# twmitchel/FieldConv

Hardware: AMD Instinct MI355X
Metric: FieldConv fwd+bwd Medges/s (20k verts, k=32, C=48, M=2) (higher is better)
Workload: dtype f32 (complex64 in/out; contractions on f16 MFMA with every operand split into two halves, fp32 accumulate)

## Files before the change

### fieldconv_amd/build.py

```python
import os
import shutil
import subprocess
import sys

PKG = os.path.dirname(os.path.abspath(__file__))
CSRC = os.path.join(PKG, 'csrc')
OUT_DIR = os.path.join(PKG, '_native')
LIB_PATH = os.path.join(OUT_DIR, 'libfieldconv_hip.so')
SOURCES = ['fc_api.hip', 'fc_pack.hip', 'fc_forward.hip', 'fc_forward_split.hip', 'fc_forward_ring.hip', 'fc_backward.hip', 'fc_backward_split.hip', 'fc_generic.hip', 'fc_cgemm.hip', 'fc_wide.hip', 'fc_blocks.hip', 'fc_pointwise.hip', 'fc_pointwise_f64.hip', 'fc_echo.hip', 'fc_trans_field.hip', 'fc_lift_echo_generic.hip', 'fc_head.hip', 'fc_graph.hip', 'fc_precomp.hip', 'fc_optim.hip', 'fc_support.hip', 'fc_loss.hip', 'fc_segment.hip', 'fc_match.hip', 'fc_linear_ce.hip', 'fc_geodesic.hip', 'fc_geodesic_fps.hip', 'fc_logmap.hip', 'fc_mesh_graph.hip', 'fc_transfer.hip', 'fc_norm.hip', 'fc_interp.hip', 'fc_maxpool.hip', 'fc_dropout.hip', 'fc_augment.hip']
HEADERS = ['fc_common.hpp', 'fc_pair.hpp', 'fc_kernels.hpp', 'fc_tile.hpp', 'fc_forward_kernels.hpp', 'fc_forward_ring.hpp', 'fc_backward_kernels.hpp', 'fc_backward_stream.hpp', 'fc_geodesic_relax.hpp', 'fc_segment.hpp', 'fc_select.hpp', 'fc_workspace.hpp', 'fc_philox.hpp', os.path.join('..', '..', 'include', 'fieldconv_hip.h')]
FLAGS = ['-O3', '-std=c++17', '--offload-arch=gfx950', '-fPIC', '-shared', '-fno-slp-vectorize',
         '-fno-gpu-rdc', '-Wno-unused-result']


def _hipcc():
    for cand in (shutil.which('hipcc'), '/opt/rocm/bin/hipcc'):
        if cand and os.path.exists(cand):
            return cand
    raise RuntimeError('hipcc not found: libfieldconv_hip.so cannot be built')


def _source_digest():
    import hashlib
    h = hashlib.sha256()
    for d in [os.path.join(CSRC, s) for s in SOURCES + HEADERS] + [os.path.abspath(__file__)]:
# ... 150 lines not shown
```

### fieldconv_amd/csrc/fc_backward.hip

```cpp
#include <stdio.h>
#include "fc_backward_kernels.hpp"
#include "fc_backward_stream.hpp"

namespace fc {

template <int T>
__global__ __launch_bounds__(kThreads) void fc_backward_filter_kernel(
    const float2* __restrict__ gx_, const float* __restrict__ hdump, float2* __restrict__ ggwp ,
    const BwdArgs a, const int F, const int B) {
    extern __shared__ __attribute__((aligned(16))) char smem[];
    const MmaGeom& mg = a.g;
    const int KD = a.KD, KP = mg.KP, IP = mg.MP, I = a.I;
    float* const slab0 = reinterpret_cast<float*>(smem);
    float* const xtr = slab0 + 2 * a.slab_stride;
    float* const xts = xtr + IP * kXtStride;
    float* const xtd = xts + IP * kXtStride;

    const int tid = threadIdx.x;
    const int lane = tid & 63;
    const int wave = __builtin_amdgcn_readfirstlane(tid >> 6);
    const int f = blockIdx.y;
    const int m = f - B;
    const int fr = lane & 15, fq = lane >> 4;

// ... 490 lines not shown
    }
    const float sc = 1.f / (float)F;
    int r = k / O, o = k - r * O;
    if (pairs == 2) {
        o = k / R;
        r = k - o * R;
    } else if (pairs && k < (R >> 1) * 2 * O) {
        const int pr = k / (2 * O), rem = k - pr * 2 * O;
        r = 2 * pr + (rem & 1);
        o = rem >> 1;
    }
    gw[(((size_t)o * I + i) * R + r) * F + f] = make_float2(s.x * sc, s.y * sc);
}

template <int R, int B>
static int launch_gather(const float2* gy, const float* rec, const fc_csr* g, const float* wpk, char* hrec, const StreamArgs& a,
                         const StreamPlan& p, hipStream_t stream) {
    const size_t lds = (size_t)p.gwpg * kRingChunks * 1024;
    if (p.gwpg == kGatherSmallWaves)
        hipLaunchKernelGGL((fc_backward_gather_kernel<R, B, kGatherSmallWaves, kGatherSmallResidency>), dim3(p.ggrid), dim3(kGatherSmallWaves * kWave),
                           lds, stream, gy, rec, g->rowptr, g->runs, wpk, hrec, a);
    else
        hipLaunchKernelGGL((fc_backward_gather_kernel<R, B, kWaves, kWaves / 4>), dim3(p.ggrid), dim3(kThreads), lds, stream, gy, rec, g->rowptr,
                           g->runs, wpk, hrec, a);
    return hipGetLastError() == hipSuccess ? FC_OK : FC_ERR_LAUNCH;
}

template <int T, int KPT = 0, int IT = 0>
static int launch_stream(const float2* x, const char* hrec, const float* wpk, float2* gwp, float2* gxt, const StreamArgs& a,
                         const StreamPlan& p, hipStream_t stream) {
    auto kern = fc_backward_stream_kernel<T, KPT, IT>;
    static bool lds_ok[kMaxDevices] = {};
    if (!allow_full_lds(reinterpret_cast<const void*>(kern), p.lds, lds_ok)) return FC_ERR_LAUNCH;
    hipLaunchKernelGGL(kern, dim3(p.P, p.FS), dim3(kThreads), p.lds, stream, x, hrec, wpk, gwp, gxt, a);
    return hipGetLastError() == hipSuccess ? FC_OK : FC_ERR_LAUNCH;
}

int backward_stream_impl(const float* x, const float* gy, const float* rec, const fc_csr* g, const float* wpk, float* gx, void* ws,
                         size_t ws_bytes, const fc_dims* d, hipStream_t stream, int stages) {
    const StreamPlan p = plan_stream(d, halves_of(d), true);
    if (!p.ok) return FC_ERR_UNSUPPORTED;
    if (!ws || ws_bytes < p.hrec_bytes + p.gwp_bytes + p.gxt_bytes + p.wst_bytes) return FC_ERR_WORKSPACE;
    StreamArgs a = make_stream_args(d, p);
    char* hrec = static_cast<char*>(ws);
    a.wst = reinterpret_cast<uint32_t*>(hrec + p.hrec_bytes + p.gwp_bytes + p.gxt_bytes);
    float2* gwp = reinterpret_cast<float2*>(hrec + p.hrec_bytes);
    float2* gxt = reinterpret_cast<float2*>(hrec + p.hrec_bytes + p.gwp_bytes);
    const float2* x2 = reinterpret_cast<const float2*>(x);
    int rc = FC_ERR_UNSUPPORTED;
    if (stages & 1) {
        const float2* gy2 = reinterpret_cast<const float2*>(gy);
#define FC_GATHER_CASE(RR, BB) if (d->R == RR && d->B == BB) rc = launch_gather<RR, BB>(gy2, rec, g, wpk, hrec, a, p, stream);
        FC_GATHER_CASE(2, 1) FC_GATHER_CASE(4, 1) FC_GATHER_CASE(6, 1) FC_GATHER_CASE(8, 1)
        FC_GATHER_CASE(2, 2) FC_GATHER_CASE(4, 2) FC_GATHER_CASE(6, 2) FC_GATHER_CASE(8, 2)
        FC_GATHER_CASE(2, 3) FC_GATHER_CASE(4, 3) FC_GATHER_CASE(6, 3) FC_GATHER_CASE(8, 3)
#undef FC_GATHER_CASE
        if (rc != FC_OK) return rc;
    }
    if (!(stages & 2)) return FC_OK;
    if (p.T == 6 && p.KPS == 288 && d->I == 48) rc = launch_stream<6, 288, 48>(x2, hrec, wpk, gwp, gxt, a, p, stream);
    else if (p.T == 6 && p.KPS == 192 && d->I == 64) rc = launch_stream<6, 192, 64>(x2, hrec, wpk, gwp, gxt, a, p, stream);
    else if (p.T <= 2) rc = launch_stream<2>(x2, hrec, wpk, gwp, gxt, a, p, stream);
    else if (p.T <= 4) rc = launch_stream<4>(x2, hrec, wpk, gwp, gxt, a, p, stream);
    else rc = launch_stream<6>(x2, hrec, wpk, gwp, gxt, a, p, stream);
    if (rc != FC_OK || (stages & 4)) return rc;
    const size_t count = (size_t)d->N * d->I;
    const dim3 grid((unsigned)((count + 255) / 256));
    float2* gx2 = reinterpret_cast<float2*>(gx);
    if (d->B == 1) hipLaunchKernelGGL(fc_backward_gx_kernel<1>, grid, dim3(256), 0, stream, x2, gxt, gx2, count, p.KS);
    else if (d->B == 2) hipLaunchKernelGGL(fc_backward_gx_kernel<2>, grid, dim3(256), 0, stream, x2, gxt, gx2, count, p.KS);
    else hipLaunchKernelGGL(fc_backward_gx_kernel<3>, grid, dim3(256), 0, stream, x2, gxt, gx2, count, p.KS);
    return hipGetLastError() == hipSuccess ? FC_OK : FC_ERR_LAUNCH;
}

bool backward_streams(const fc_dims* d, bool factored) { return plan_stream(d, halves_of(d), factored).ok; }

bool backward_fits(const fc_dims* d) { return plan_backward(d, halves_of(d)).ok_factored; }

size_t backward_workspace_bytes(const fc_dims* d) {
    const BwdPlan p = plan_backward(d, halves_of(d));
    const size_t pair = p.hdump_bytes + p.gwp_bytes + p.gxp_bytes + 256;
    const StreamPlan sp = plan_stream(d, halves_of(d), true);
    const size_t stream = sp.ok ? sp.hrec_bytes + sp.gwp_bytes + sp.gxt_bytes + sp.wst_bytes + 256 : 0;
    return pair > stream ? pair : stream;
}

template <int T>
static int launch_backward_filter(const float2* x, const float* hdump, float2* gwp, const BwdArgs& a, const BwdPlan& p,
                                  const fc_dims* d, hipStream_t stream) {
    static const bool half2 = !(dev_env("FC_FILTER2") && atoi(dev_env("FC_FILTER2")) == 0);
    static bool ok_half2[kMaxDevices] = {}, ok_half[kMaxDevices] = {}, ok_f32[kMaxDevices] = {};
    if (p.fhalf && half2) {
        const size_t lds2 = (size_t)(2 * kTile * filter_image_stride(p.KP) + 2 * 6 * p.IP * kXbStride + 8) * sizeof(_Float16) + 16;
        static bool ok_half2h[kMaxDevices] = {};
        if (a.dump_halves) {
            if (!allow_full_lds(reinterpret_cast<const void*>(fc_backward_filter_half2_kernel<T, true>), lds2, ok_half2h)) return FC_ERR_LAUNCH;
            hipLaunchKernelGGL((fc_backward_filter_half2_kernel<T, true>), dim3(p.P, p.F), dim3(kThreads), lds2, stream, x, hdump, gwp, a, p.F,
                               d->B, d->R * d->O);
// ... 28 lines not shown
        const int per_col = kWaves / p.g.NMT, row_tiles = p.KP / 16;
        need = (row_tiles + per_col - 1) / per_col;
    }
    if (need <= 2) return launch_backward_filter<2>(x2, hdump, gwp, a, p, d, stream);
    if (need <= 4) return launch_backward_filter<4>(x2, hdump, gwp, a, p, d, stream);
    if (need <= 6) return launch_backward_filter<6>(x2, hdump, gwp, a, p, d, stream);
    if (need <= kMaxGwTiles) return launch_backward_filter<kMaxGwTiles>(x2, hdump, gwp, a, p, d, stream);
    return FC_ERR_UNSUPPORTED;
}

void describe_backward(const fc_dims* d, int records, char* buf, size_t n) {
    {
        const StreamPlan sp = plan_stream(d, halves_of(d), records != 0);
        if (sp.ok) {
            snprintf(buf, n, "fc_backward_gather_kernel<records,split-f16> tiles=%d (%d workgroups of %d wavefronts, %d per SIMD); fc_backward_stream_kernel (H once for gxt and gW: %d gxt + %d gW "
                     "wavefronts, W_f in registers, records by LDS-DMA) grid=%dx%d; fc_backward_gx_kernel; module parameters: "
                     "fc_backward_finish_params (sum of the partials + parameter chain) in one launch; explicit filter: fc_backward_finish; cus=%d",
                     sp.ntiles, sp.ggrid, sp.gwpg, sp.gwaves, sp.G, sp.NW, sp.P, sp.FS, num_cus());
            return;
        }
    }
    const BwdPlan p = plan_backward(d, halves_of(d));
    const char* mode = halves_of(d) == 2 ? "split-f16" : halves_of(d) == 1 ? "f16" : "f32";
    static const bool staged = [] { const char* e = dev_env("FC_FILTER2"); return e && atoi(e) == 0; }();
    static const bool split_finish = [] { const char* e = dev_env("FC_SPLIT_FINISH"); return e && atoi(e) != 0; }();
    const int gx_parts = (1 << p.parts_log2) * (p.gsplit ? 2 : 1);
    char fin[320];
    if (split_finish)
        snprintf(fin, sizeof(fin), "%sfc_backward_finish + fc_filter_param_grads (two launches: the split-finish development switch)",
                 gx_parts > 1 ? "fc_sum_parts_kernel (the partial gx arrays), " : "");
    else
// ... 72 lines not shown
```

### fieldconv_amd/csrc/fc_backward_stream.hpp

```cpp
#pragma once
#include <stdlib.h>
#include "fc_backward_kernels.hpp"

namespace fc {

constexpr int kStreamUnits = 4;
constexpr int kStreamPartStride = 2 * kTile + 4;

struct StreamPlan {
    bool ok;
    int F, KP, IP, NMT, KST, KSI, NU, G, NW, T, ntiles, P, nslots;
    int KS;
    int FS, KPS;
    int NG;
    int gwpg, gwaves;
    int ggrid;
    int img_bytes;
    int rec_bytes;
    size_t lds;
    size_t hrec_bytes, gwp_bytes, gxt_bytes, wst_bytes;
    int nt_dump;
};

struct StreamArgs {
    int N, I, O, R, F, B;
    int KP, IP, NMT, KST, KSI, G, NW, ntiles, P, nslots;
    int KS;
    int img_bytes, rec_bytes;
    int wKI, wKP;
    int nt_dump;
    uint32_t* wst;
    unsigned long long* stamps;
    unsigned long long* meter;
    int dbg;
};

constexpr int kGatherSmallWaves = 4;
constexpr int kGatherSmallResidency = 5;
inline void plan_gather(const fc_dims* d, StreamPlan& p);

inline StreamPlan plan_stream(const fc_dims* d, int halves, bool factored) {
    StreamPlan p = {};
    p.ok = false;
    static const bool off = [] { const char* e = dev_env("FC_BWD_STREAM"); return e && atoi(e) == 0; }();
    if (off || !factored || halves != 2 || d->N <= 0) return p;
    const int R = d->R, O = d->O, I = d->I;
// ... 27 lines not shown
    const int cus = num_cus();
    if (4 * p.ntiles < 3 * cus) return p;
    p.P = cus / p.FS;
    if (p.P < 1) p.P = 1;
    p.img_bytes = kTile * p.KSI * 2;
    p.rec_bytes = round_up(p.img_bytes + 2 * kTile * 4, 1024);
    if (I & 1) return p;
    p.lds = (size_t)2 * p.rec_bytes + (size_t)2 * 4 * p.IP * kXbStride * 2 + (size_t)3 * kTile * I * 8 + 4 * 64 * 4 + 2 * 8 * 64 * 4 +
            2 * 64 * 4 + (size_t)2 * p.nslots * kTile * kStreamPartStride * 4;
    if (kTile * I * 8 > kWaves * 1024 - 1024) return p;
    if ((size_t)d->N * I * 8 >= ((size_t)1 << 32)) return p;
    if (p.lds > kMaxLds) return p;
    p.hrec_bytes = (size_t)p.ntiles * p.FS * p.rec_bytes + 1024;
    p.gwp_bytes = (size_t)p.P * p.F * p.KP * p.IP * sizeof(float2);
    p.gxt_bytes = (size_t)p.FS * d->N * I * sizeof(float2);
    p.wst_bytes = (size_t)p.FS * p.G * 4 * kStreamUnits * kWave * 16;
    p.nt_dump = p.hrec_bytes > ((size_t)192 << 20) ? 1 : 0;
    plan_gather(d, p);
    p.ok = true;
    return p;
}

inline StreamArgs make_stream_args(const fc_dims* d, const StreamPlan& p) {
    StreamArgs a;
    a.N = d->N; a.I = d->I; a.O = d->O; a.R = d->R; a.F = p.FS; a.B = d->B; a.KS = p.KS;
    a.KP = p.KPS; a.IP = p.IP; a.NMT = p.NMT; a.KST = p.KST; a.KSI = p.KSI; a.G = p.G; a.NW = p.NW; a.ntiles = p.ntiles; a.P = p.P;
    a.nslots = p.nslots;
    a.img_bytes = p.img_bytes; a.rec_bytes = p.rec_bytes;
    const MmaGeom gw = make_mma_geom(d->I, d->R, d->O, 2);
    a.wKI = gw.KI; a.wKP = gw.KP;
    a.nt_dump = p.nt_dump;
    a.wst = nullptr;
    static const int dbg = [] { const char* e = dev_env("FC_DEBUG_BWD"); return e ? atoi(e) : 0; }();
    a.dbg = dbg;
    static const bool stamp_me = [] { const char* e = dev_env("FC_STAMP_KERNEL"); return e && e[0] == 's'; }();
    a.stamps = stamp_me ? debug_stamp_buffer() : nullptr;
    static const bool meter_me = [] { const char* e = dev_env("FC_STAMP_KERNEL"); return e && e[0] == 'w'; }();
    a.meter = meter_me && debug_stamp_buffer() ? debug_stamp_buffer() + kMeterGather : nullptr;
    return a;
}

typedef uint32_t u32x3 __attribute__((ext_vector_type(3)));

template <int R, bool NT>
__device__ __forceinline__ void store_plane_row(uint32_t* dst, const uint32_t (&w)[R / 2]) {
    if constexpr (R == 2) {
        if (NT) __builtin_nontemporal_store(w[0], dst); else *dst = w[0];
// ... 3 lines not shown
        if (NT) __builtin_nontemporal_store(v, reinterpret_cast<u2*>(dst)); else *reinterpret_cast<u2*>(dst) = v;
    } else if constexpr (R == 6) {
        typedef u32x3 __attribute__((aligned(4))) u3;
        const u32x3 v = {w[0], w[1], w[2]};
        if (NT) __builtin_nontemporal_store(v, reinterpret_cast<u3*>(dst)); else *reinterpret_cast<u3*>(dst) = v;
    } else {
        typedef u32x4 __attribute__((aligned(4))) u4;
        const u32x4 v = {w[0], w[1], w[2], w[3]};
        if (NT) __builtin_nontemporal_store(v, reinterpret_cast<u4*>(dst)); else *reinterpret_cast<u4*>(dst) = v;
    }
}

template <int R, int B, int WPG, int MINW>
__global__ __launch_bounds__(WPG * kWave, MINW) void fc_backward_gather_kernel(
    const float2* __restrict__ ggy, const float* __restrict__ gsten, const int32_t* __restrict__ growptr,
    const int32_t* __restrict__ gruns, const float* __restrict__ gwpk, char* __restrict__ hrec, const StreamArgs a) {
    constexpr int F = 2 * B + 1;
    static_assert(F * R <= 64 && (R & 1) == 0, "at most two walks per vertex, an even ring count");
    constexpr int NG = (F * R + 31) / 32;
    constexpr int FG = (F + NG - 1) / NG;
    constexpr int RECF = factored_record_floats(B);
    constexpr int LOG_CR = factored_log_chunk_records(B);
    constexpr int CR = 1 << LOG_CR;
    constexpr int NR = kRingChunks;
    extern __shared__ __attribute__((aligned(16))) char smem[];
    const int tid = threadIdx.x;
    const int lane = tid & 63;
    const int wave = __builtin_amdgcn_readfirstlane(tid >> 6);
    float* const ring = reinterpret_cast<float*>(smem) + wave * NR * 256;
    const int O = a.O;
    const int ol = lane < O ? lane : 0;

    auto dma_chunk = [&](const int first, const int ch) {
        uint32_t lane_off = lane;
        asm volatile("" : "+v"(lane_off));
        const char* src = reinterpret_cast<const char*>(gsten + ((size_t)first + ((size_t)ch << LOG_CR)) * RECF) + lane_off * 16u;
        __builtin_amdgcn_global_load_lds((gptr_t)src, (lptr_t)(ring + (ch & (NR - 1)) * 256), 16, 0, 0);
    };
    auto slot_range = [&](const int item, int& b, int& e, int (&run)[R]) {
        b = 0;
        e = 0;
#pragma unroll
        for (int q = 0; q < R; ++q) run[q] = 0;
// ... 160 lines not shown
                        float* tail = reinterpret_cast<float*>(recf + half_off + (uint32_t)a.img_bytes);
                        tail[row] = scale;
                        tail[kTile + row] = inv_scale;
                    }
                }
            };
            if (a.nt_dump && !(kDevSwitches && (a.dbg & 32))) rows(std::true_type{}); else rows(std::false_type{});
        });
        beg = nbeg;
        end = nend;
#pragma unroll
        for (int q = 0; q < R; ++q) ro[q] = nro[q];
    }

    meter.close();

    {
        const int total = a.F * a.G * kStreamUnits * 4 * kWave;
        const int NU = a.NMT * a.KST;
        const size_t plane_sz = (size_t)a.IP * a.wKP;
        const uint16_t* const img0 = reinterpret_cast<const uint16_t*>(gwpk + a.IP);
        for (int e = (blockIdx.x * WPG + wave) * kWave + lane; e < total; e += gridDim.x * (WPG * kWave)) {
            const int ln = e & 63, pl = (e >> 6) & 3, ui = (e >> 8) % kStreamUnits, fg = e / (kStreamUnits * 4 * kWave);
            const int g_ = fg % a.G, sl = fg / a.G;
            const int f_ = sl / a.KS, k0 = (sl - f_ * a.KS) * a.KP;
            const int fr_ = ln & 15, fq_ = ln >> 4;
            const int u = min(g_ * kStreamUnits + ui, NU - 1);
            const int mt = u / a.KST, kb = u - mt * a.KST;
            const int row = (mt * 16 + fr_) * 32;
            const uint16_t* const img = img0 + ((size_t)f_ * 4 + pl) * plane_sz;
            int o = (k0 + kb * 32 + 8 * fq_) / R, r = k0 + kb * 32 + 8 * fq_ - o * R;
            uint32_t v[4];
#pragma unroll
            for (int jj = 0; jj < 4; ++jj) {
                uint32_t pr[2];
#pragma unroll
                for (int e2 = 0; e2 < 2; ++e2) {
                    const int kk = r * a.wKI + o;
                    pr[e2] = img[(size_t)(kk >> 5) * a.IP * 32 + row + (kk & 31)];
                    if (++r == R) { r = 0; ++o; }
                }
                v[jj] = pr[0] | (pr[1] << 16);
            }
            *reinterpret_cast<u32x4*>(a.wst + (size_t)e * 4) = u32x4{v[0], v[1], v[2], v[3]};
        }
    }
}

template <int R, int B>
inline bool gather_fits_small() {
    static const bool fits = [] {
        hipFuncAttributes at;
        const void* fn = reinterpret_cast<const void*>(fc_backward_gather_kernel<R, B, kGatherSmallWaves, kGatherSmallResidency>);
        if (hipFuncGetAttributes(&at, fn) != hipSuccess) {
            (void)hipGetLastError();
            return false;
        }
        return at.localSizeBytes == 0 && at.numRegs <= (512 / kGatherSmallResidency) / 8 * 8;
    }();
    return fits;
}
// ... 197 lines not shown
        stamp(10);
        asm volatile("s_waitcnt vmcnt(0) lgkmcnt(0)" ::: "memory");
        stamp(0);
        __builtin_amdgcn_s_barrier();
        stamp(2);
        requests(k + 1, k + 3, a.G);
        stamp(4);
        stamp(1);
    };

    if (is_gxt) {
        const int u0 = wave * kStreamUnits;
        const int NU = a.NMT * a.KST;
        u32x4 wrh[kStreamUnits], wrl[kStreamUnits], wih[kStreamUnits], wil[kStreamUnits];
        {
            const u32x4* const ws = reinterpret_cast<const u32x4*>(a.wst) + (size_t)(f * a.G + wave) * (kStreamUnits * 4 * kWave) + lane;
#pragma unroll
            for (int ui = 0; ui < kStreamUnits; ++ui) {
                wrh[ui] = ws[(ui * 4 + 0) * kWave];
                wrl[ui] = ws[(ui * 4 + 1) * kWave];
                wih[ui] = ws[(ui * 4 + 2) * kWave];
                wil[ui] = ws[(ui * 4 + 3) * kWave];
            }
        }
        first_requests();
#pragma unroll
        for (int ui = 0; ui < kStreamUnits; ++ui) asm volatile("" : "+v"(wrh[ui]), "+v"(wrl[ui]), "+v"(wih[ui]), "+v"(wil[ui]));
        const int hbase = fr * KSI + 8 * fq;
        for (int k = 0; k < nrec; ++k) {
            head(k);
            if (k > 0) reduce_gxt(k - 1);
            const lds_f16* const img = (const lds_f16*)(smem + (k & 1) * a.rec_bytes) + hbase;
            if (!(kDevSwitches && (a.dbg & 2))) {
                float* const pp = part0 + (k & 1) * part_floats + (4 * fq) * kStreamPartStride + 2 * fr;
                const float isv = tail0[(k & 3) * 64 + kTile + fr];
                f32x4 are = {0.f, 0.f, 0.f, 0.f}, aim = are, arn = are;
                int mt_prev = u0 / a.KST;
// ... 152 lines not shown
```

### fieldconv_amd/csrc/fc_kernels.hpp

```cpp
#pragma once
#include <hip/hip_runtime.h>
#include "../../include/fieldconv_hip.h"

#define FC_FOR_EACH_SHAPE(X) \
    X(2, 1) X(3, 1) X(4, 1) X(5, 1) X(6, 1) X(7, 1) X(8, 1) \
    X(2, 2) X(3, 2) X(4, 2) X(5, 2) X(6, 2) X(7, 2) X(8, 2) \
    X(2, 3) X(3, 3) X(4, 3) X(5, 3) X(6, 3) X(7, 3) X(8, 3)

namespace fc {

constexpr size_t kMaxLds = 160 * 1024;
constexpr int kDefaultCUs = 256;
constexpr int kMaxDevices = 16;
inline int num_cus() {
    static int cached[kMaxDevices] = {};
    int dev = 0;
    if (hipGetDevice(&dev) != hipSuccess || dev < 0) return kDefaultCUs;
    if (dev < kMaxDevices && cached[dev] > 0) return cached[dev];
    int n = 0;
    if (hipDeviceGetAttribute(&n, hipDeviceAttributeMultiprocessorCount, dev) != hipSuccess || n <= 0) n = kDefaultCUs;
    if (dev < kMaxDevices) cached[dev] = n;
    return n;
}
constexpr int kMaxChannels = 64;

int forward_impl(const float* x, const float* sten, const fc_csr* g, const float* wpk, float* y,
                 const fc_dims* d, int kind, void* ws, size_t ws_bytes, const fc_epilogue* epi, hipStream_t stream);
size_t forward_workspace_bytes(const fc_dims* d, int kind);
size_t backward_workspace_bytes(const fc_dims* d);
int backward_data_impl(const float* x, const float* gy, const float* sten, const fc_csr* g, const float* wpk, float* gx,
                       void* ws, size_t ws_bytes, const fc_dims* d, bool factored, hipStream_t stream, bool defer_gx_sum = false);
int backward_filter_impl(const float* x, void* ws, size_t ws_bytes, const fc_dims* d, hipStream_t stream, bool factored = false);
bool backward_streams(const fc_dims* d, bool factored);
int backward_stream_impl(const float* x, const float* gy, const float* rec, const fc_csr* g, const float* wpk, float* gx, void* ws,
                         size_t ws_bytes, const fc_dims* d, hipStream_t stream, int stages);
int backward_finish_impl(float* gw_eff, void* ws, size_t ws_bytes, const fc_dims* d, hipStream_t stream, bool factored = false);
int pack_filter_impl(const float* w_eff, float* wpk_fwd, float* wpk_bwd, const fc_dims* d, int records, hipStream_t stream);
int pack_filter_params_impl(const float* zonal, const float* sph, const float* phase, int ftype, float* wpk_fwd,
                            float* wpk_bwd, const fc_dims* d, int records, hipStream_t stream);
int pack_filter_params_pair_impl(const fc_filter_params& f0, float* fwd0, float* bwd0, const fc_dims* d0, const fc_filter_params& f1,
                                 float* fwd1, float* bwd1, const fc_dims* d1, int records, hipStream_t stream);
size_t packed_filter_floats_fwd(const fc_dims* d, int records);
size_t packed_filter_floats_bwd(const fc_dims* d, int records);

bool ring_enabled(const fc_dims* d);
bool forward_ring_fits(const fc_dims* d);
size_t packed_ring_image_floats(int M, int F, int channels, int R, int halves);
int forward_ring_impl(const float* x, const float* rec, const fc_csr* g, const float* wpk, float* y, const fc_dims* d, int kind,
// ... 49 lines not shown
```

### fieldconv_amd/csrc/fc_pack.hip

```cpp
#include <stdlib.h>
#include "fc_common.hpp"
#include "fc_kernels.hpp"
#include "fc_tile.hpp"
#include "fc_forward_ring.hpp"

namespace fc {

__device__ __forceinline__ float2 filter_entry(const float* __restrict__ zonal, const float* __restrict__ sph,
                                               const float* __restrict__ phase, int ftype, int B, int R, int I, int o, int i,
                                               int r, int f) {
    const size_t oir = ((size_t)o * I + i) * R + r;
    if (ftype == 2) {
        if (f == B) return make_float2(zonal[oir * 2], zonal[oir * 2 + 1]);
        const int b = f < B ? f : f - 1;
        const float* p = sph + (oir * (2 * B) + b) * 2;
        return make_float2(p[0], p[1]);
    }
    const int q = f >= B ? f - B : B - f;
    const float z = zonal[oir];
    float2 sp = make_float2(0.f, 0.f);
    if (B > 0) sp = *reinterpret_cast<const float2*>(sph + (oir * B + (q > 0 ? q - 1 : 0)) * 2);
    float ph = 0.f;
    if (ftype == 1) ph = phase[((size_t)o * I + i) * (B + 1) + q];
    float2 c = q == 0 ? make_float2(z, 0.f) : make_float2(sp.x, f > B ? sp.y : -sp.y);
    if (ftype == 1) {
        float s, co;
        sincosf(ph, &s, &co);
        c = cmul(c, make_float2(co, s));
    }
    return c;
}

struct PackArgs {
    int O, I, R, F, B, ftype;
    MmaGeom gf, gb;
    unsigned blocks_f;
    int ring_f;
    int o0, i0, Ifull;
};

constexpr int kPackThreads = 256;

template <bool FROM_PARAMS, bool WITH_PHASE>
__device__ __forceinline__ float2 packed_value(const float2* __restrict__ w, const float* __restrict__ zonal,
                                               const float* __restrict__ sph, const float* __restrict__ phase,
                                               const PackArgs& a, bool is_bwd, int m, int k, int slab) {
    const int KI = is_bwd ? a.gb.KI : a.gf.KI;
    const bool ring = !is_bwd && a.ring_f;
    const int kk = k / KI, c = k - kk * KI;
    const int r = ring ? slab : kk, f = ring ? kk : slab;
    if (f >= a.F) return make_float2(0.f, 0.f);
    const int o = is_bwd ? c : m, i = is_bwd ? m : c;
    if (o >= a.O || i >= a.I || r >= a.R) return make_float2(0.f, 0.f);
    const float2 v = FROM_PARAMS ? filter_entry(zonal, sph, phase, (!WITH_PHASE && a.ftype == 1) ? 0 : a.ftype, a.B, a.R, a.Ifull, a.o0 + o,
                                                a.i0 + i, r, f)
                                 : w[(((size_t)(a.o0 + o) * a.Ifull + a.i0 + i) * a.R + r) * a.F + f];
// ... 46 lines not shown
    const unsigned blk = is_bwd ? block - a.blocks_f : block;
    const MmaGeom& g = is_bwd ? a.gb : a.gf;
    float* const img = is_bwd ? bwd : fwd;
    if (!g.split) {
        const size_t j = (size_t)blk * kPackThreads + threadIdx.x;
        if (j >= (size_t)a.F * 2 * g.MP * g.KP) return;
        const int k = j % g.KP;
        const int m = (j / g.KP) % g.MP;
        const int pl = (j / ((size_t)g.KP * g.MP)) % 2;
        const int f = j / ((size_t)g.KP * g.MP * 2);
        const float2 v = packed_value<FROM_PARAMS, true>(w, zonal, sph, phase, a, is_bwd, m, k, f);
        img[j] = pl == 0 ? v.x : v.y;
        return;
    }
    __shared__ float red[kPackThreads / kWave];
    const int nslab = (!is_bwd && a.ring_f) ? a.R : a.F;
    const int m = blk / nslab, f = blk - m * nslab;
    float mx = row_max2<FROM_PARAMS>(w, zonal, sph, a, is_bwd, m);
#pragma unroll
    for (int d = 32; d >= 1; d >>= 1) mx = fmaxf(mx, __shfl_xor(mx, d, 64));
    if ((threadIdx.x & 63) == 0) red[threadIdx.x >> 6] = mx;
    __syncthreads();
    mx = sqrtf(fmaxf(fmaxf(red[0], red[1]), fmaxf(red[2], red[3]))) * 1.0000002f;
    float scale, inv;
    split_scale(mx, scale, inv);
    if (threadIdx.x == 0 && f == 0) img[m] = inv;
    _Float16* const planes = reinterpret_cast<_Float16*>(img + g.MP);
    const size_t plane = (size_t)g.MP * g.KP;
    for (int k = threadIdx.x; k < g.KP; k += kPackThreads) {
        const float2 v = packed_value<FROM_PARAMS, true>(w, zonal, sph, phase, a, is_bwd, m, k, f);
        _Float16 rh, rl, ih, il;
        split_halves(v.x * scale, rh, rl);
        split_halves(v.y * scale, ih, il);
        _Float16* p = planes + (size_t)f * 2 * g.split * plane + ((size_t)(k >> 5) * g.MP + m) * 32 + (k & 31);
        if (g.split == 2) {
            p[0] = rh;
            p[plane] = rl;
            p[2 * plane] = ih;
            p[3 * plane] = il;
        } else {
            p[0] = rh;
            p[plane] = ih;
        }
    }
}

template <bool FROM_PARAMS>
__global__ __launch_bounds__(kPackThreads) void fc_pack_filter_kernel(const float2* __restrict__ w, const float* __restrict__ zonal,
                                                                      const float* __restrict__ sph,
                                                                      const float* __restrict__ phase, float* __restrict__ fwd,
                                                                      float* __restrict__ bwd, const PackArgs a) {
    pack_filter_body<FROM_PARAMS>(w, zonal, sph, phase, fwd, bwd, a, blockIdx.x);
}

struct PackPtrs { const float* zonal; const float* sph; const float* phase; float* fwd; float* bwd; };
__global__ __launch_bounds__(kPackThreads) void fc_pack_filter_pair_kernel(const PackPtrs p0, const PackArgs a0, const PackPtrs p1,
                                                                           const PackArgs a1, const unsigned split) {
    if (blockIdx.x < split) pack_filter_body<true>(nullptr, p0.zonal, p0.sph, p0.phase, p0.fwd, p0.bwd, a0, blockIdx.x);
    else pack_filter_body<true>(nullptr, p1.zonal, p1.sph, p1.phase, p1.fwd, p1.bwd, a1, blockIdx.x - split);
// ... 8 lines not shown
size_t packed_filter_floats_fwd(const fc_dims* d, int records) {
    if (ring_forward_image(d, records)) return packed_ring_image_floats(d->O, 2 * d->B + 1, d->I, d->R, halves_of(d));
    return packed_image_floats(d->O, d->R, d->I, 2 * d->B + 1, halves_of(d));
}
size_t packed_filter_floats_bwd(const fc_dims* d, int records) {
    (void)records;
    return packed_image_floats(d->I, d->R, d->O, 2 * d->B + 1, halves_of(d));
}

static unsigned pack_args(PackArgs& a, int ftype, bool want_fwd, bool want_bwd, const fc_dims* d, int records, int o0, int i0, int Ifull) {
    a.O = d->O; a.I = d->I; a.R = d->R; a.B = d->B; a.F = 2 * d->B + 1; a.ftype = ftype;
    a.o0 = o0; a.i0 = i0; a.Ifull = Ifull > 0 ? Ifull : d->I;
    a.ring_f = ring_forward_image(d, records & 1) ? 1 : 0;
    a.gf = a.ring_f ? ring_geom(d->O, a.F, d->I, halves_of(d)) : make_mma_geom(d->O, d->R, d->I, halves_of(d));
    a.gb = make_mma_geom(d->I, d->R, d->O, halves_of(d));
    a.blocks_f = want_fwd ? pack_blocks(a.gf, a.ring_f ? a.R : a.F) : 0u;
    const unsigned blocks_b = pack_blocks(a.gb, a.F);
    return a.blocks_f + (want_bwd ? blocks_b : 0u);
}

int pack_filter_params_pair_impl(const fc_filter_params& f0, float* fwd0, float* bwd0, const fc_dims* d0, const fc_filter_params& f1,
                                 float* fwd1, float* bwd1, const fc_dims* d1, int records, hipStream_t stream) {
    PackArgs a0, a1;
    const unsigned n0 = pack_args(a0, f0.ftype, fwd0 != nullptr, bwd0 != nullptr, d0, records, 0, 0, 0);
    const unsigned n1 = pack_args(a1, f1.ftype, fwd1 != nullptr, bwd1 != nullptr, d1, records, 0, 0, 0);
    if (n0 == 0 || n1 == 0) return FC_ERR_BAD_ARGUMENT;
    const PackPtrs p0{f0.zonal, f0.spherical, f0.phase, fwd0, bwd0}, p1{f1.zonal, f1.spherical, f1.phase, fwd1, bwd1};
    hipLaunchKernelGGL(fc_pack_filter_pair_kernel, dim3(n0 + n1), dim3(kPackThreads), 0, stream, p0, a0, p1, a1, n0);
    return hipGetLastError() == hipSuccess ? FC_OK : FC_ERR_LAUNCH;
}
// ... 247 lines not shown
```

### fieldconv_amd/functional.py

```python
import ctypes
import os

import torch

from . import _lib
from ._launch import NO_GUARD as _NO_GUARD, _dp, _p, _po, by_value as _by_value, carve as _carve, on as _on, scratch as _scratch, stream as _stream
from ._lib import FcCsr, FcDims, FcEpilogue, FcFilterParams, check


class KernelTimer:

    def __init__(self):
        self.enabled = False
        self.stride = 1
        self.events = {}
        self.count = {}
        self.pool = []

    def reset(self, pairs=0):
        self.events = {}
        self.count = {}
        self.pool = [(torch.cuda.Event(enable_timing=True), torch.cuda.Event(enable_timing=True)) for _ in range(pairs)]

    def elapsed_ms(self):
# ... 94 lines not shown
@_lib.keep_mode
class _FieldConvFn(torch.autograd.Function):

    @staticmethod
    def forward(ctx, x, w_eff, graph):
        lib = _lib.load()
        x = _by_value(x)
        w_eff = _by_value(w_eff)
        O, I, R, F = w_eff.shape
        B = (F - 1) // 2
        plan = _conv_plan(lib, graph, I, O, B)
        with _on(x.device):
            st = _stream()

            def pack(pl, wpk_f, wpk_b):
                check(lib.fc_pack_filter(_p(w_eff), _p(wpk_f), _po(wpk_b), pl.dref, pl.records, st), 'fc_pack_filter')
            y, wpk_b = _run_forward(lib, x, graph, plan, O, st, pack)
        ctx.save_for_backward(x, wpk_b)
        ctx.graph = graph
        ctx.wshape = (O, I, R, F)
        return y

    @staticmethod
    def backward(ctx, gy):
        lib = _lib.load()
        x, wpk_b = ctx.saved_tensors
        O, I, R, F = ctx.wshape
        plan = _conv_plan(lib, ctx.graph, I, O, (F - 1) // 2)
        gy = _by_value(gy)
        with _on(x.device):
            gx, gw, _ = _launch_backward(lib, x, gy, ctx.graph, wpk_b, plan, ctx.wshape, _stream())
# ... 95 lines not shown
            kind, recs, _ = _records(graph)
            check(lib.fc_forward_params(_p(x), _p(recs), plan.cref_t, kind, ctypes.byref(_filter_params(params)), _p(wpk_f), _p(wpk_b), _p(y),
                                        _po(ws), plan.ws_fwd, plan.dref, plan.records, epi, st), 'fc_forward_params')
            return (y if bias is None else (y, act)), wpk_b
        pack(plan, wpk_f, wpk_b)
        if between is not None:
            between()
        return _launch_forward(lib, x, graph, wpk_f, plan, O, st, addend=addend, bias=bias), wpk_b
    y = torch.empty((nt, O), dtype=torch.complex64, device=dev)
    act = torch.empty_like(y) if bias is not None else None
    if len(ranges) == 1 and between is not None:
        between()
    for row0, nrows in ranges:
        sub = _row_plan(lib, graph, plan, row0, nrows)
        wpk_f = torch.empty(sub.n_fwd, dtype=torch.float32, device=dev)
        pack(sub, wpk_f, wpk_b if row0 == 0 else None)
        _launch_forward(lib, x, graph, wpk_f, sub, O, st, addend=addend, bias=bias, out=(y, act), row0=row0)
        if row0 == 0 and len(ranges) == 2:
            between()
    return (y if bias is None else (y, act)), wpk_b


def _param_grads(params):
    zonal, spherical, phase, ftype = params
    return torch.empty_like(zonal), torch.empty_like(spherical), (torch.empty_like(phase) if ftype == 1 else None)


def _launch_backward(lib, x, gy, graph, wpk_b, plan, wshape, st, params=None, bias_sum=None):
    O, I, R, F = wshape
    gx = torch.empty_like(x)
    want_gw = params is None or KEEP_GW_EFF or _split_finish()
# ... 31 lines not shown
    if graph.on_gx is not None:
        graph.on_gx(gx)
    with _timed('fc_backward_filter'):
        check(lib.fc_backward_filter(_p(x), wsp, nbytes, plan.dref, plan.records, st), 'fc_backward_filter')
    if fp is not None:
        check(lib.fc_backward_finish_params(gwp, wsp, nbytes, plan.dref, plan.records, ctypes.byref(fp), st), 'fc_backward_finish_params')
    else:
        check(lib.fc_backward_finish(_p(gw), wsp, nbytes, plan.dref, plan.records, st), 'fc_backward_finish')
    return gx, gw, pgrads


def _param_packer(lib, params, st):
    zonal, spherical, phase, ftype = params

    def pack(pl, wpk_f, wpk_b):
        check(lib.fc_pack_filter_params(_p(zonal), _p(spherical), _p(phase), ftype, _p(wpk_f), _po(wpk_b), pl.dref, pl.records, st),
              'fc_pack_filter_params')
    return pack


@_lib.keep_mode
class _FieldConvParamFn(torch.autograd.Function):

    @staticmethod
    def forward(ctx, x, zonal, spherical, phase, ftype, B, graph):
        lib = _lib.load()
        x = _by_value(x)
        zonal, spherical, phase = _by_value(zonal), _by_value(spherical, 8), _by_value(phase)
        O, I, R = zonal.shape[0], zonal.shape[1], zonal.shape[2]
        F = 2 * B + 1
        plan = _conv_plan(lib, graph, I, O, B)
# ... 695 lines not shown
```

Baseline: 1824.

## Write backward filter fragments in MMA order during packing, drop gather-kernel reshuffle

The filter-packing kernel now stages the backward split-f16 planes in LDS and writes them directly in the per-lane fragment order that the backward stream kernel loads into registers. The gather kernel no longer carries a tail loop that rebuilt this fragment table from the packed image on every backward pass. The stream kernel reads the fragments straight from the packed filter buffer. This removes scattered 16-bit reads and an extra workspace write from backward, in exchange for LDS staging and an extra pack call for the backward filter when rows are split.

```diff
diff --git a/fieldconv_amd/build.py b/fieldconv_amd/build.py
--- a/fieldconv_amd/build.py
+++ b/fieldconv_amd/build.py
@@ -8,7 +8,7 @@
 OUT_DIR = os.path.join(PKG, '_native')
 LIB_PATH = os.path.join(OUT_DIR, 'libfieldconv_hip.so')
 SOURCES = ['fc_api.hip', 'fc_pack.hip', 'fc_forward.hip', 'fc_forward_split.hip', 'fc_forward_ring.hip', 'fc_backward.hip', 'fc_backward_split.hip', 'fc_generic.hip', 'fc_cgemm.hip', 'fc_wide.hip', 'fc_blocks.hip', 'fc_pointwise.hip', 'fc_pointwise_f64.hip', 'fc_echo.hip', 'fc_trans_field.hip', 'fc_lift_echo_generic.hip', 'fc_head.hip', 'fc_graph.hip', 'fc_precomp.hip', 'fc_optim.hip', 'fc_support.hip', 'fc_loss.hip', 'fc_segment.hip', 'fc_match.hip', 'fc_linear_ce.hip', 'fc_geodesic.hip', 'fc_geodesic_fps.hip', 'fc_logmap.hip', 'fc_mesh_graph.hip', 'fc_transfer.hip', 'fc_norm.hip', 'fc_interp.hip', 'fc_maxpool.hip', 'fc_dropout.hip', 'fc_augment.hip']
-HEADERS = ['fc_common.hpp', 'fc_pair.hpp', 'fc_kernels.hpp', 'fc_tile.hpp', 'fc_forward_kernels.hpp', 'fc_forward_ring.hpp', 'fc_backward_kernels.hpp', 'fc_backward_stream.hpp', 'fc_geodesic_relax.hpp', 'fc_segment.hpp', 'fc_select.hpp', 'fc_workspace.hpp', 'fc_philox.hpp', os.path.join('..', '..', 'include', 'fieldconv_hip.h')]
+HEADERS = ['fc_common.hpp', 'fc_pair.hpp', 'fc_kernels.hpp', 'fc_tile.hpp', 'fc_forward_kernels.hpp', 'fc_forward_ring.hpp', 'fc_backward_kernels.hpp', 'fc_backward_stream.hpp', 'fc_stream_frag.hpp', 'fc_geodesic_relax.hpp', 'fc_segment.hpp', 'fc_select.hpp', 'fc_workspace.hpp', 'fc_philox.hpp', os.path.join('..', '..', 'include', 'fieldconv_hip.h')]
 FLAGS = ['-O3', '-std=c++17', '--offload-arch=gfx950', '-fPIC', '-shared', '-fno-slp-vectorize',
          '-fno-gpu-rdc', '-Wno-unused-result']
 
diff --git a/fieldconv_amd/csrc/fc_backward.hip b/fieldconv_amd/csrc/fc_backward.hip
--- a/fieldconv_amd/csrc/fc_backward.hip
+++ b/fieldconv_amd/csrc/fc_backward.hip
@@ -528,15 +528,15 @@
 }
 
 template <int R, int B>
-static int launch_gather(const float2* gy, const float* rec, const fc_csr* g, const float* wpk, char* hrec, const StreamArgs& a,
+static int launch_gather(const float2* gy, const float* rec, const fc_csr* g, char* hrec, const StreamArgs& a,
                          const StreamPlan& p, hipStream_t stream) {
     const size_t lds = (size_t)p.gwpg * kRingChunks * 1024;
     if (p.gwpg == kGatherSmallWaves)
         hipLaunchKernelGGL((fc_backward_gather_kernel<R, B, kGatherSmallWaves, kGatherSmallResidency>), dim3(p.ggrid), dim3(kGatherSmallWaves * kWave),
-                           lds, stream, gy, rec, g->rowptr, g->runs, wpk, hrec, a);
+                           lds, stream, gy, rec, g->rowptr, g->runs, hrec, a);
     else
         hipLaunchKernelGGL((fc_backward_gather_kernel<R, B, kWaves, kWaves / 4>), dim3(p.ggrid), dim3(kThreads), lds, stream, gy, rec, g->rowptr,
-                           g->runs, wpk, hrec, a);
+                           g->runs, hrec, a);
     return hipGetLastError() == hipSuccess ? FC_OK : FC_ERR_LAUNCH;
 }
 
@@ -554,17 +554,17 @@
                          size_t ws_bytes, const fc_dims* d, hipStream_t stream, int stages) {
     const StreamPlan p = plan_stream(d, halves_of(d), true);
     if (!p.ok) return FC_ERR_UNSUPPORTED;
-    if (!ws || ws_bytes < p.hrec_bytes + p.gwp_bytes + p.gxt_bytes + p.wst_bytes) return FC_ERR_WORKSPACE;
+    if (!ws || ws_bytes < p.hrec_bytes + p.gwp_bytes + p.gxt_bytes + p.spare_bytes) return FC_ERR_WORKSPACE;
     StreamArgs a = make_stream_args(d, p);
     char* hrec = static_cast<char*>(ws);
-    a.wst = reinterpret_cast<uint32_t*>(hrec + p.hrec_bytes + p.gwp_bytes + p.gxt_bytes);
+    a.wst = reinterpret_cast<const uint32_t*>(wpk + stream_frag_offset_floats(d));
     float2* gwp = reinterpret_cast<float2*>(hrec + p.hrec_bytes);
     float2* gxt = reinterpret_cast<float2*>(hrec + p.hrec_bytes + p.gwp_bytes);
     const float2* x2 = reinterpret_cast<const float2*>(x);
     int rc = FC_ERR_UNSUPPORTED;
     if (stages & 1) {
         const float2* gy2 = reinterpret_cast<const float2*>(gy);
-#define FC_GATHER_CASE(RR, BB) if (d->R == RR && d->B == BB) rc = launch_gather<RR, BB>(gy2, rec, g, wpk, hrec, a, p, stream);
+#define FC_GATHER_CASE(RR, BB) if (d->R == RR && d->B == BB) rc = launch_gather<RR, BB>(gy2, rec, g, hrec, a, p, stream);
         FC_GATHER_CASE(2, 1) FC_GATHER_CASE(4, 1) FC_GATHER_CASE(6, 1) FC_GATHER_CASE(8, 1)
         FC_GATHER_CASE(2, 2) FC_GATHER_CASE(4, 2) FC_GATHER_CASE(6, 2) FC_GATHER_CASE(8, 2)
         FC_GATHER_CASE(2, 3) FC_GATHER_CASE(4, 3) FC_GATHER_CASE(6, 3) FC_GATHER_CASE(8, 3)
@@ -589,13 +589,19 @@
 
 bool backward_streams(const fc_dims* d, bool factored) { return plan_stream(d, halves_of(d), factored).ok; }
 
+bool backward_stream_frag(const fc_dims* d, bool factored, StreamFrag* frag) {
+    const StreamPlan p = plan_stream(d, halves_of(d), factored);
+    if (p.ok && frag) *frag = p.frag;
+    return p.ok;
+}
+
 bool backward_fits(const fc_dims* d) { return plan_backward(d, halves_of(d)).ok_factored; }
 
 size_t backward_workspace_bytes(const fc_dims* d) {
     const BwdPlan p = plan_backward(d, halves_of(d));
     const size_t pair = p.hdump_bytes + p.gwp_bytes + p.gxp_bytes + 256;
     const StreamPlan sp = plan_stream(d, halves_of(d), true);
-    const size_t stream = sp.ok ? sp.hrec_bytes + sp.gwp_bytes + sp.gxt_bytes + sp.wst_bytes + 256 : 0;
+    const size_t stream = sp.ok ? sp.hrec_bytes + sp.gwp_bytes + sp.gxt_bytes + sp.spare_bytes + 256 : 0;
     return pair > stream ? pair : stream;
 }
 
@@ -654,7 +660,7 @@
         const StreamPlan sp = plan_stream(d, halves_of(d), records != 0);
         if (sp.ok) {
             snprintf(buf, n, "fc_backward_gather_kernel<records,split-f16> tiles=%d (%d workgroups of %d wavefronts, %d per SIMD); fc_backward_stream_kernel (H once for gxt and gW: %d gxt + %d gW "
-                     "wavefronts, W_f in registers, records by LDS-DMA) grid=%dx%d; fc_backward_gx_kernel; module parameters: "
+                     "wavefronts, W_f in registers from the fragment-order filter the packing launch wrote, records by LDS-DMA) grid=%dx%d; fc_backward_gx_kernel; module parameters: "
                      "fc_backward_finish_params (sum of the partials + parameter chain) in one launch; explicit filter: fc_backward_finish; cus=%d",
                      sp.ntiles, sp.ggrid, sp.gwpg, sp.gwaves, sp.G, sp.NW, sp.P, sp.FS, num_cus());
             return;
diff --git a/fieldconv_amd/csrc/fc_backward_stream.hpp b/fieldconv_amd/csrc/fc_backward_stream.hpp
--- a/fieldconv_amd/csrc/fc_backward_stream.hpp
+++ b/fieldconv_amd/csrc/fc_backward_stream.hpp
@@ -1,10 +1,10 @@
 #pragma once
 #include <stdlib.h>
 #include "fc_backward_kernels.hpp"
+#include "fc_stream_frag.hpp"
 
 namespace fc {
 
-constexpr int kStreamUnits = 4;
 constexpr int kStreamPartStride = 2 * kTile + 4;
 
 struct StreamPlan {
@@ -18,7 +18,9 @@
     int img_bytes;
     int rec_bytes;
     size_t lds;
-    size_t hrec_bytes, gwp_bytes, gxt_bytes, wst_bytes;
+    size_t hrec_bytes, gwp_bytes, gxt_bytes;
+    StreamFrag frag;
+    size_t spare_bytes;
     int nt_dump;
 };
 
@@ -29,7 +31,8 @@
     int img_bytes, rec_bytes;
     int wKI, wKP;
     int nt_dump;
-    uint32_t* wst;
+    const uint32_t* wst;
+    StreamFrag frag;
     unsigned long long* stamps;
     unsigned long long* meter;
     int dbg;
@@ -87,7 +90,8 @@
     p.hrec_bytes = (size_t)p.ntiles * p.FS * p.rec_bytes + 1024;
     p.gwp_bytes = (size_t)p.P * p.F * p.KP * p.IP * sizeof(float2);
     p.gxt_bytes = (size_t)p.FS * d->N * I * sizeof(float2);
-    p.wst_bytes = (size_t)p.FS * p.G * 4 * kStreamUnits * kWave * 16;
+    p.frag = StreamFrag{R, p.FS, p.KS, p.KPS, p.KST, p.NU};
+    p.spare_bytes = (size_t)p.FS * p.G * 4 * kStreamUnits * kWave * 16;
     p.nt_dump = p.hrec_bytes > ((size_t)192 << 20) ? 1 : 0;
     plan_gather(d, p);
     p.ok = true;
@@ -104,6 +108,7 @@
     a.wKI = gw.KI; a.wKP = gw.KP;
     a.nt_dump = p.nt_dump;
     a.wst = nullptr;
+    a.frag = p.frag;
     static const int dbg = [] { const char* e = dev_env("FC_DEBUG_BWD"); return e ? atoi(e) : 0; }();
     a.dbg = dbg;
     static const bool stamp_me = [] { const char* e = dev_env("FC_STAMP_KERNEL"); return e && e[0] == 's'; }();
@@ -137,7 +142,7 @@
 template <int R, int B, int WPG, int MINW>
 __global__ __launch_bounds__(WPG * kWave, MINW) void fc_backward_gather_kernel(
     const float2* __restrict__ ggy, const float* __restrict__ gsten, const int32_t* __restrict__ growptr,
-    const int32_t* __restrict__ gruns, const float* __restrict__ gwpk, char* __restrict__ hrec, const StreamArgs a) {
+    const int32_t* __restrict__ gruns, char* __restrict__ hrec, const StreamArgs a) {
     constexpr int F = 2 * B + 1;
     static_assert(F * R <= 64 && (R & 1) == 0, "at most two walks per vertex, an even ring count");
     constexpr int NG = (F * R + 31) / 32;
@@ -147,9 +152,8 @@
     constexpr int CR = 1 << LOG_CR;
     constexpr int NR = kRingChunks;
     extern __shared__ __attribute__((aligned(16))) char smem[];
-    const int tid = threadIdx.x;
-    const int lane = tid & 63;
-    const int wave = __builtin_amdgcn_readfirstlane(tid >> 6);
+    const int lane = threadIdx.x & 63;
+    const int wave = __builtin_amdgcn_readfirstlane(threadIdx.x >> 6);
     float* const ring = reinterpret_cast<float*>(smem) + wave * NR * 256;
     const int O = a.O;
     const int ol = lane < O ? lane : 0;
@@ -340,37 +344,6 @@
     }
 
     meter.close();
-
-    {
-        const int total = a.F * a.G * kStreamUnits * 4 * kWave;
-        const int NU = a.NMT * a.KST;
-        const size_t plane_sz = (size_t)a.IP * a.wKP;
-        const uint16_t* const img0 = reinterpret_cast<const uint16_t*>(gwpk + a.IP);
-        for (int e = (blockIdx.x * WPG + wave) * kWave + lane; e < total; e += gridDim.x * (WPG * kWave)) {
-            const int ln = e & 63, pl = (e >> 6) & 3, ui = (e >> 8) % kStreamUnits, fg = e / (kStreamUnits * 4 * kWave);
-            const int g_ = fg % a.G, sl = fg / a.G;
-            const int f_ = sl / a.KS, k0 = (sl - f_ * a.KS) * a.KP;
-            const int fr_ = ln & 15, fq_ = ln >> 4;
-            const int u = min(g_ * kStreamUnits + ui, NU - 1);
-            const int mt = u / a.KST, kb = u - mt * a.KST;
-            const int row = (mt * 16 + fr_) * 32;
-            const uint16_t* const img = img0 + ((size_t)f_ * 4 + pl) * plane_sz;
-            int o = (k0 + kb * 32 + 8 * fq_) / R, r = k0 + kb * 32 + 8 * fq_ - o * R;
-            uint32_t v[4];
-#pragma unroll
-            for (int jj = 0; jj < 4; ++jj) {
-                uint32_t pr[2];
-#pragma unroll
-                for (int e2 = 0; e2 < 2; ++e2) {
-                    const int kk = r * a.wKI + o;
-                    pr[e2] = img[(size_t)(kk >> 5) * a.IP * 32 + row + (kk & 31)];
-                    if (++r == R) { r = 0; ++o; }
-                }
-                v[jj] = pr[0] | (pr[1] << 16);
-            }
-            *reinterpret_cast<u32x4*>(a.wst + (size_t)e * 4) = u32x4{v[0], v[1], v[2], v[3]};
-        }
-    }
 }
 
 template <int R, int B>
@@ -598,13 +571,14 @@
         const int NU = a.NMT * a.KST;
         u32x4 wrh[kStreamUnits], wrl[kStreamUnits], wih[kStreamUnits], wil[kStreamUnits];
         {
-            const u32x4* const ws = reinterpret_cast<const u32x4*>(a.wst) + (size_t)(f * a.G + wave) * (kStreamUnits * 4 * kWave) + lane;
+            const u32x4* const ws = reinterpret_cast<const u32x4*>(a.wst) + stream_frag_entry(a.frag, f, 0, 0, lane);
 #pragma unroll
             for (int ui = 0; ui < kStreamUnits; ++ui) {
-                wrh[ui] = ws[(ui * 4 + 0) * kWave];
-                wrl[ui] = ws[(ui * 4 + 1) * kWave];
-                wih[ui] = ws[(ui * 4 + 2) * kWave];
-                wil[ui] = ws[(ui * 4 + 3) * kWave];
+                const u32x4* const wu = ws + stream_frag_step(stream_frag_slot_unit(a.frag, wave, ui), 0);
+                wrh[ui] = wu[stream_frag_step(0, 0)];
+                wrl[ui] = wu[stream_frag_step(0, 1)];
+                wih[ui] = wu[stream_frag_step(0, 2)];
+                wil[ui] = wu[stream_frag_step(0, 3)];
             }
         }
         first_requests();
diff --git a/fieldconv_amd/csrc/fc_kernels.hpp b/fieldconv_amd/csrc/fc_kernels.hpp
--- a/fieldconv_amd/csrc/fc_kernels.hpp
+++ b/fieldconv_amd/csrc/fc_kernels.hpp
@@ -32,6 +32,8 @@
                        void* ws, size_t ws_bytes, const fc_dims* d, bool factored, hipStream_t stream, bool defer_gx_sum = false);
 int backward_filter_impl(const float* x, void* ws, size_t ws_bytes, const fc_dims* d, hipStream_t stream, bool factored = false);
 bool backward_streams(const fc_dims* d, bool factored);
+struct StreamFrag;
+bool backward_stream_frag(const fc_dims* d, bool factored, StreamFrag* frag);
 int backward_stream_impl(const float* x, const float* gy, const float* rec, const fc_csr* g, const float* wpk, float* gx, void* ws,
                          size_t ws_bytes, const fc_dims* d, hipStream_t stream, int stages);
 int backward_finish_impl(float* gw_eff, void* ws, size_t ws_bytes, const fc_dims* d, hipStream_t stream, bool factored = false);
diff --git a/fieldconv_amd/csrc/fc_pack.hip b/fieldconv_amd/csrc/fc_pack.hip
--- a/fieldconv_amd/csrc/fc_pack.hip
+++ b/fieldconv_amd/csrc/fc_pack.hip
@@ -3,6 +3,7 @@
 #include "fc_kernels.hpp"
 #include "fc_tile.hpp"
 #include "fc_forward_ring.hpp"
+#include "fc_stream_frag.hpp"
 
 namespace fc {
 
@@ -36,10 +37,14 @@
     MmaGeom gf, gb;
     unsigned blocks_f;
     int ring_f;
+    int frag_on;
+    StreamFrag frag;
+    size_t frag_off;
     int o0, i0, Ifull;
 };
 
 constexpr int kPackThreads = 256;
+constexpr int kPackStage = 8 * kMaxChannels;
 
 template <bool FROM_PARAMS, bool WITH_PHASE>
 __device__ __forceinline__ float2 packed_value(const float2* __restrict__ w, const float* __restrict__ zonal,
@@ -116,6 +121,8 @@
         return;
     }
     __shared__ float red[kPackThreads / kWave];
+    __shared__ __attribute__((aligned(16))) _Float16 stage[4][kPackStage];
+    const bool frag = is_bwd && a.frag_on;
     const int nslab = (!is_bwd && a.ring_f) ? a.R : a.F;
     const int m = blk / nslab, f = blk - m * nslab;
     float mx = row_max2<FROM_PARAMS>(w, zonal, sph, a, is_bwd, m);
@@ -135,7 +142,16 @@
         split_halves(v.x * scale, rh, rl);
         split_halves(v.y * scale, ih, il);
         _Float16* p = planes + (size_t)f * 2 * g.split * plane + ((size_t)(k >> 5) * g.MP + m) * 32 + (k & 31);
-        if (g.split == 2) {
+        if (frag) {
+            const int r = k / g.KI, o = k - r * g.KI;
+            if (r < a.R && o < a.O) {
+                const int ko = o * a.R + r;
+                stage[0][ko] = rh;
+                stage[1][ko] = rl;
+                stage[2][ko] = ih;
+                stage[3][ko] = il;
+            }
+        } else if (g.split == 2) {
             p[0] = rh;
             p[plane] = rl;
             p[2 * plane] = ih;
@@ -145,6 +161,16 @@
             p[plane] = ih;
         }
     }
+    if (frag) {
+        __syncthreads();
+        u32x4* const dst = reinterpret_cast<u32x4*>(img + a.frag_off);
+        const int n8 = a.R * a.O / 8;
+        for (int t = threadIdx.x; t < 4 * n8; t += kPackThreads) {
+            const int pl = t / n8, k8 = (t - pl * n8) * 8;
+            const u32x4 v = *reinterpret_cast<const u32x4*>(&stage[pl][k8]);
+            dst[stream_frag_entry_of(a.frag, f, m, k8, pl)] = v;
+        }
+    }
 }
 
 template <bool FROM_PARAMS>
@@ -183,6 +209,9 @@
     a.ring_f = ring_forward_image(d, records & 1) ? 1 : 0;
     a.gf = a.ring_f ? ring_geom(d->O, a.F, d->I, halves_of(d)) : make_mma_geom(d->O, d->R, d->I, halves_of(d));
     a.gb = make_mma_geom(d->I, d->R, d->O, halves_of(d));
+    a.frag = StreamFrag{};
+    a.frag_on = (want_bwd && backward_stream_frag(d, records != 0, &a.frag)) ? 1 : 0;
+    a.frag_off = stream_frag_offset_floats(d);
     a.blocks_f = want_fwd ? pack_blocks(a.gf, a.ring_f ? a.R : a.F) : 0u;
     const unsigned blocks_b = pack_blocks(a.gb, a.F);
     return a.blocks_f + (want_bwd ? blocks_b : 0u);
diff --git a/fieldconv_amd/csrc/fc_stream_frag.hpp b/fieldconv_amd/csrc/fc_stream_frag.hpp
--- /dev/null
+++ b/fieldconv_amd/csrc/fc_stream_frag.hpp
@@ -0,0 +1,32 @@
+#pragma once
+#include <cstddef>
+#include <cstdint>
+#include "fc_common.hpp"
+#include "fc_tile.hpp"
+
+namespace fc {
+
+constexpr int kStreamUnits = 4;
+
+struct StreamFrag {
+    int R, FS, KS, KPS, KST, NU;
+};
+
+__host__ __device__ constexpr int stream_frag_step(int unit, int plane) { return (unit * 4 + plane) * kWave; }
+__host__ __device__ inline size_t stream_frag_entry(const StreamFrag& g, int slice, int unit, int plane, int lane) {
+    return (size_t)slice * stream_frag_step(g.NU, 0) + stream_frag_step(unit, plane) + lane;
+}
+__host__ __device__ inline int stream_frag_slot_unit(const StreamFrag& g, int wave, int ui) {
+    const int u = wave * kStreamUnits + ui;
+    return u < g.NU ? u : g.NU - 1;
+}
+__host__ __device__ inline size_t stream_frag_bytes(const StreamFrag& g) { return stream_frag_entry(g, g.FS, 0, 0, 0) * 16; }
+
+__host__ __device__ inline size_t stream_frag_entry_of(const StreamFrag& g, int f, int i, int k8, int plane) {
+    const int h = k8 / g.KPS, kk = k8 - h * g.KPS;
+    return stream_frag_entry(g, f * g.KS + h, (i >> 4) * g.KST + kk / 32, plane, 16 * ((kk & 31) >> 3) + (i & 15));
+}
+
+inline size_t stream_frag_offset_floats(const fc_dims* d) { return (size_t)round_up(d->I, 16); }
+
+}
diff --git a/fieldconv_amd/functional.py b/fieldconv_amd/functional.py
--- a/fieldconv_amd/functional.py
+++ b/fieldconv_amd/functional.py
@@ -132,7 +132,7 @@
             st = _stream()
 
             def pack(pl, wpk_f, wpk_b):
-                check(lib.fc_pack_filter(_p(w_eff), _p(wpk_f), _po(wpk_b), pl.dref, pl.records, st), 'fc_pack_filter')
+                check(lib.fc_pack_filter(_p(w_eff), _po(wpk_f), _po(wpk_b), pl.dref, pl.records, st), 'fc_pack_filter')
             y, wpk_b = _run_forward(lib, x, graph, plan, O, st, pack)
         ctx.save_for_backward(x, wpk_b)
         ctx.graph = graph
@@ -258,7 +258,9 @@
     for row0, nrows in ranges:
         sub = _row_plan(lib, graph, plan, row0, nrows)
         wpk_f = torch.empty(sub.n_fwd, dtype=torch.float32, device=dev)
-        pack(sub, wpk_f, wpk_b if row0 == 0 else None)
+        pack(sub, wpk_f, None)
+        if row0 == 0:
+            pack(plan, None, wpk_b)
         _launch_forward(lib, x, graph, wpk_f, sub, O, st, addend=addend, bias=bias, out=(y, act), row0=row0)
         if row0 == 0 and len(ranges) == 2:
             between()
@@ -320,7 +322,7 @@
     zonal, spherical, phase, ftype = params
 
     def pack(pl, wpk_f, wpk_b):
-        check(lib.fc_pack_filter_params(_p(zonal), _p(spherical), _p(phase), ftype, _p(wpk_f), _po(wpk_b), pl.dref, pl.records, st),
+        check(lib.fc_pack_filter_params(_p(zonal), _p(spherical), _p(phase), ftype, _po(wpk_f), _po(wpk_b), pl.dref, pl.records, st),
               'fc_pack_filter_params')
     return pack
 
```

Result: no change. 1818 (-0.3%).
